# hiroharu-kato/neural_renderer

Measured on AMD Instinct MI355X. Metric: rasterize fwd+bwd Mpixels/sec @256x256 batch=64, higher is better.
Workload: dtype f32

## Files before the change

neural_renderer_amd/csrc/nr_device.h:

```cpp
#pragma once
#include <hip/hip_runtime.h>
#include <stdint.h>
#include <stdlib.h>

#include "../../include/nr_hip.h"

#define NR_API extern "C" __attribute__((visibility("default")))

namespace nr {

constexpr int WAVE = 64;


__device__ __forceinline__ bool is_backside(float x0, float y0, float x1, float y1, float x2, float y2)
{
    return (y2 - y0) * (x1 - x0) < (y1 - y0) * (x2 - x0);
}

__device__ __forceinline__ float to_pixel(float v, float fs) { return 0.5f * (v * fs + fs - 1.0f); }

__device__ __forceinline__ void compute_face_inv(const float px[3], const float py[3], float inv[9])
{
    inv[0] = py[1] - py[2];
    inv[1] = px[2] - px[1];
// ... 69 lines not shown
    if (thin || wild) {
        c.bw = S; c.n = S * S;
        return c;
    }
    const float xmin = fminf(fminf(px[0], px[1]), px[2]), xmax = fmaxf(fmaxf(px[0], px[1]), px[2]);
    const float ymin = fminf(fminf(py[0], py[1]), py[2]), ymax = fmaxf(fmaxf(py[0], py[1]), py[2]);
    const float lo_c = -2.0f, hi_c = (float)S + 1.0f;
    const int xl = max((int)ceilf(fminf(fmaxf(xmin - BBOX_GUARD, lo_c), hi_c)), 0);
    const int xh = min((int)floorf(fminf(fmaxf(xmax + BBOX_GUARD, lo_c), hi_c)), S - 1);
    const int yl = max((int)ceilf(fminf(fmaxf(ymin - BBOX_GUARD, lo_c), hi_c)), 0);
    const int yh = min((int)floorf(fminf(fmaxf(ymax + BBOX_GUARD, lo_c), hi_c)), S - 1);
    if (xl <= xh && yl <= yh) {
        c.x_lo = xl; c.y_lo = yl; c.bw = xh - xl + 1; c.n = c.bw * (yh - yl + 1);
    }
    return c;
}

__device__ __forceinline__ bool cand_pixel(const Cand &c, int i, int S, int &x, int &y)
{
    if (c.strip == 0) {
        const int yy = i / c.bw;
        x = c.x_lo + (i - yy * c.bw);
        y = c.y_lo + yy;
        return true;
    }
    const int m = i / STRIP_W, j = i - m * STRIP_W;
    const int o = (int)floorf(c.a * (float)m + c.b) - 1 + j;
    if (c.strip == 1) { y = m; x = o; } else { x = m; y = o; }
    return o >= 0 && o < S;
}

struct FaceLight {
    const float *light = nullptr;
    int tex_faces = 0;
    const float *textures = nullptr;
    float *grad_light = nullptr;
};

__device__ __forceinline__ int transpose_texel(int t, int ts)
{
    const int k = t % ts, j = (t / ts) % ts, i = t / (ts * ts);
    return (k * ts + j) * ts + i;
}

struct Taps {
    int isc[8];
    float w[8];
};

__device__ __forceinline__ void compute_taps(const float *__restrict__ z, const float *__restrict__ weight,
                                             float depth, int ts, double eps, Taps &t, bool flip = false)
{
    float tif[3];
    int ti[3];
    float fr[3];
#pragma unroll
    for (int k = 0; k < 3; k++) {
        float v = weight[k] * (float)(ts - 1) * (depth / z[k]);
        v = fmaxf(v, 0.0f);
        v = (float)fmin((double)v, (double)(ts - 1) - eps);
        tif[k] = v;
        ti[k] = (int)v;
        fr[k] = v - (float)ti[k];
    }
#pragma unroll
    for (int pn = 0; pn < 8; pn++) {
        float w = 1.0f;
        int idx[3];
#pragma unroll
        for (int k = 0; k < 3; k++) {
            if (((pn >> k) & 1) == 0) {
                w *= 1.0f - fr[k];
                idx[k] = ti[k];
            } else {
                w *= fr[k];
                idx[k] = ti[k] + 1;
            }
        }
        t.isc[pn] = (flip ? idx[2] : idx[0]) * ts * ts + idx[1] * ts + (flip ? idx[0] : idx[2]);
        t.w[pn] = w;
    }
}


__device__ __forceinline__ int f2i(float x) { return (int)x; }

__device__ __forceinline__ void texel_reads(const float *face, const float d[3], int H, int W, long long p[4], float w[4])
{
    const float pos_x = (face[0] * d[0] + face[2] * d[1] + face[4] * d[2]) * (float)(W - 1);
    const float pos_y = (face[1] * d[0] + face[3] * d[1] + face[5] * d[2]) * (float)(H - 1);
    const int xi = f2i(pos_x), yi = f2i(pos_y), yi1 = f2i(pos_y + 1.0f);
    const float wx1 = pos_x - (float)xi, wx0 = 1.0f - wx1;
    const float wy1 = pos_y - (float)yi, wy0 = 1.0f - wy1;
    const long long last = (long long)H * W - 1;
    auto clampi = [&](int row, int col) -> long long {
        const long long q = (long long)row * W + col;
        return q < 0 ? 0 : (q > last ? last : q);
    };
    p[0] = clampi(yi, xi);
    p[1] = clampi(yi1, xi);
    p[2] = clampi(yi, xi + 1);
    p[3] = clampi(yi1, xi + 1);
    w[0] = wx0 * wy0;
    w[1] = wx0 * wy1;
    w[2] = wx1 * wy0;
    w[3] = wx1 * wy1;
}

__device__ __forceinline__ int mirror_row(long long p, int H, int W)
{
    const int row = (int)(p / W), col = (int)(p - (long long)row * W);
    return (H - 1 - row) * W + col;
}

struct UVShade {
    const float *images = nullptr;
    const int32_t *table = nullptr;
    const float *faces_uv = nullptr;
    const int32_t *face_image = nullptr;
    const float *base = nullptr;
    int ts = 0, M = 0, P = 0;
    int shared = 0;
};

struct UVSample {
    int m, f0;
    int q[4];
    float w[4];
    Taps t;
};

__device__ __forceinline__ void corner_weights(const float (&z)[3], const float (&w)[3], float zp, float (&d)[3])
{
#pragma unroll
    for (int k = 0; k < 3; k++) d[k] = fminf(fmaxf(w[k] * (zp / z[k]), 0.0f), 1.0f);
}

__device__ __forceinline__ void uv_locate(const UVShade &uv, int fi, int tex_faces, const float *face, float w0, float w1,
                                          float w2, float zp, double eps, UVSample &s)
{
    const bool flip = fi >= tex_faces;
    s.f0 = flip ? fi - tex_faces : fi;
    const int m = uv.face_image[s.f0];
    s.m = (m >= 0 && m < uv.M) ? m : -1;
    const float fz[3] = {face[2], face[5], face[8]};
    const float w[3] = {w0, w1, w2};
    if (s.m < 0) {
        compute_taps(fz, w, zp, uv.ts, eps, s.t, flip);
        return;
    }
    float d[3];
#pragma unroll
    for (int k = 0; k < 3; k++) d[k] = fminf(fmaxf(w[k] * (zp / fz[k]), 0.0f), 1.0f);
    if (flip) {
        const float d0 = d[0];
        d[0] = d[2];
        d[2] = d0;
    }
    const int off = uv.table[3 * s.m], H = uv.table[3 * s.m + 1], W = uv.table[3 * s.m + 2];
    long long p[4];
    texel_reads(uv.faces_uv + (size_t)s.f0 * 6, d, H, W, p, s.w);
#pragma unroll
    for (int r = 0; r < 4; r++) s.q[r] = off + mirror_row(p[r], H, W);
}

__device__ __forceinline__ void uv_color(const UVShade &uv, const UVSample &s, int b, float c[3])
// ... 175 lines not shown
```

neural_renderer_amd/csrc/nr_forward.hip:

```cpp
#include "nr_device.h"

using namespace nr;

namespace {

constexpr size_t SMALL_LAUNCH_FACES = (size_t)16384 * 32;
constexpr int SMALL_AREA = 256;
constexpr int WAVE_AREA = 4096;
constexpr unsigned long long ZEMPTY = ~0ull;
constexpr int QSHARDS = 16;
constexpr int QSTRIDE = 32;

__device__ __forceinline__ unsigned depth_key(float zp)
{
    const unsigned u = __float_as_uint(zp + 0.0f);
    return (u & 0x80000000u) ? ~u : (u | 0x80000000u);
}

__device__ __forceinline__ unsigned long long zword(float zp, unsigned fn, int epoch)
{
    const unsigned long long k = depth_key(zp);
    return epoch < 0 ? (k << 32) | fn : ((unsigned long long)(unsigned)epoch << 56) | (k << 24) | fn;
}

struct FaceGeo {
    float x0, y0, z0, x1, y1, z1, x2, y2, z2, i0, i1, i2, i3, i4, i5, i6, i7, i8;
};

__device__ __forceinline__ bool inside_edges(const FaceGeo &q, float xp, float yp)
{
    return !(((yp - q.y0) * (q.x1 - q.x0) < (xp - q.x0) * (q.y1 - q.y0)) ||
             ((yp - q.y1) * (q.x2 - q.x1) < (xp - q.x1) * (q.y2 - q.y1)) ||
             ((yp - q.y2) * (q.x0 - q.x2) < (xp - q.x2) * (q.y0 - q.y2)));
}

__device__ __forceinline__ bool eval_inside(const FaceGeo &q, float xif, float yif, double near_d, double far_d, float &zp,
                                            float &w0, float &w1, float &w2)
{
    w0 = q.i0 * xif + q.i1 * yif + q.i2;
    w1 = q.i3 * xif + q.i4 * yif + q.i5;
    w2 = q.i6 * xif + q.i7 * yif + q.i8;
    w0 = fminf(fmaxf(w0, 0.0f), 1.0f);
    w1 = fminf(fmaxf(w1, 0.0f), 1.0f);
    w2 = fminf(fmaxf(w2, 0.0f), 1.0f);
    const float w_sum = (0.0f + w0) + w1 + w2;
    w0 /= w_sum;
    w1 /= w_sum;
    w2 /= w_sum;
    zp = 1.0f / (w0 / q.z0 + w1 / q.z1 + w2 / q.z2);
    if ((double)zp <= near_d || far_d <= (double)zp) return false;
    return zp < (float)far_d;
}

__device__ __forceinline__ bool eval_pixel(const FaceGeo &q, float xp, float yp, float xif, float yif, double near_d,
                                           double far_d, float &zp, float &w0, float &w1, float &w2)
{
    return inside_edges(q, xp, yp) && eval_inside(q, xif, yif, near_d, far_d, zp, w0, w1, w2);
}

__device__ __forceinline__ float pixel_center_f(int i, int S) { return (float)(2 * i + 1 - S) / (float)S; }
__device__ __forceinline__ float pixel_center_p(int i, int S, float inv_s, bool pow2)
{
    return pow2 ? (float)(2 * i + 1 - S) * inv_s : (float)(2 * i + 1 - S) / (float)S;
}

__device__ __forceinline__ void load_face_geo(const float *__restrict__ f, int S, FaceGeo &g, float inv[9])
{
    g.x0 = f[0]; g.y0 = f[1]; g.z0 = f[2]; g.x1 = f[3]; g.y1 = f[4]; g.z1 = f[5]; g.x2 = f[6]; g.y2 = f[7]; g.z2 = f[8];
    if (is_backside(g.x0, g.y0, g.x1, g.y1, g.x2, g.y2)) {
#pragma unroll
        for (int k = 0; k < 9; k++) inv[k] = 0.0f;
    } else {
        const float fs = (float)S;
        const float px[3] = {to_pixel(g.x0, fs), to_pixel(g.x1, fs), to_pixel(g.x2, fs)};
        const float py[3] = {to_pixel(g.y0, fs), to_pixel(g.y1, fs), to_pixel(g.y2, fs)};
        compute_face_inv(px, py, inv);
    }
    g.i0 = inv[0]; g.i1 = inv[1]; g.i2 = inv[2]; g.i3 = inv[3]; g.i4 = inv[4]; g.i5 = inv[5];
    g.i6 = inv[6]; g.i7 = inv[7]; g.i8 = inv[8];
}

constexpr int FR_ROWS = 128;
constexpr int FR_PIX = 256;
static_assert(SMALL_AREA <= 256, "rows and columns of a kept box are packed into 8 bits each");

template <int FACES>
struct FaceWaveLds {
    float g[18][FACES];
    int x_lo[FACES], y_lo[FACES], bw[FACES], img[FACES], fn[FACES];
    int rows[FR_ROWS];
    int pix[FR_PIX];
};

__device__ __forceinline__ int wave_inclusive_sum(int v)
{
    v += __builtin_amdgcn_update_dpp(0, v, 0x111, 0xf, 0xf, true);
    v += __builtin_amdgcn_update_dpp(0, v, 0x112, 0xf, 0xf, true);
    v += __builtin_amdgcn_update_dpp(0, v, 0x114, 0xf, 0xf, true);
    v += __builtin_amdgcn_update_dpp(0, v, 0x118, 0xf, 0xf, true);
    v += __builtin_amdgcn_update_dpp(0, v, 0x142, 0xa, 0xf, false);
    v += __builtin_amdgcn_update_dpp(0, v, 0x143, 0xc, 0xf, false);
    return v;
}

__device__ __forceinline__ void wave_lds_sync()
{
    __builtin_amdgcn_fence(__ATOMIC_RELEASE, "wavefront");
    __builtin_amdgcn_wave_barrier();
    __builtin_amdgcn_fence(__ATOMIC_ACQUIRE, "wavefront");
}

template <int FACES>
__device__ __forceinline__ bool slot_pixel(const FaceWaveLds<FACES> &L, int e, int S, double near_d, double far_d,
                                           unsigned long long *__restrict__ zbuf, unsigned long long &key,
                                           unsigned long long *&at, int epoch)
{
    const int s = e >> 16;
    FaceGeo q;
    q.z0 = L.g[6][s]; q.z1 = L.g[7][s]; q.z2 = L.g[8][s];
    q.i0 = L.g[9][s]; q.i1 = L.g[10][s]; q.i2 = L.g[11][s]; q.i3 = L.g[12][s]; q.i4 = L.g[13][s];
    q.i5 = L.g[14][s]; q.i6 = L.g[15][s]; q.i7 = L.g[16][s]; q.i8 = L.g[17][s];
    const int x = L.x_lo[s] + (e & 255), y = L.y_lo[s] + ((e >> 8) & 255);
    float zp, w0, w1, w2;
    const bool ok = eval_inside(q, (float)x, (float)y, near_d, far_d, zp, w0, w1, w2);
    key = zword(zp, (unsigned)L.fn[s], epoch);
    at = zbuf + ((size_t)L.img[s] * S + y) * S + x;
    return ok;
}


template <bool POW2, int FACES, int GROUP>
__global__ __launch_bounds__(256) void k_face_raster(const float *__restrict__ faces,
                                                     unsigned long long *__restrict__ zbuf,
                                                     int *__restrict__ large_list, int *__restrict__ wave_list,
                                                     int *__restrict__ n_large, int qcap, int nshards,
                                                     unsigned char *__restrict__ visible_faces, int n_faces_total, int F,
                                                     int S, double near_d, double far_d, int epoch,
                                                     unsigned char *__restrict__ touched)
{
    __shared__ FaceWaveLds<FACES> lds[4];
    FaceWaveLds<FACES> &L = lds[threadIdx.x >> 6];
    const int lane = threadIdx.x & 63;
    const int t = blockIdx.x * blockDim.x + threadIdx.x;
    if (t < n_faces_total && visible_faces) visible_faces[t] = 0;
    const int n_waves = (n_faces_total + FACES - 1) / FACES;
    const int i = ((lane / GROUP) * n_waves + (t >> 6)) * GROUP + (lane % GROUP);
    const bool live = lane < FACES && (t >> 6) < n_waves && i < n_faces_total;
    float f[9];
    {
        float *stage = &L.g[0][0];
        const size_t n_words = (size_t)n_faces_total * 9;
        constexpr int NLOAD = (9 * FACES + 63) / 64;
        float word[NLOAD];
#pragma unroll
        for (int k = 0; k < NLOAD; k++) {
            const int d = k * 64 + lane, run = d / (9 * GROUP), off = d - run * (9 * GROUP);
            const size_t src = ((size_t)run * n_waves + (t >> 6)) * (9 * GROUP) + off;
            const float v = faces[src < n_words ? src : n_words - 1];
            word[k] = src < n_words ? v : 0.0f;
        }
#pragma unroll
        for (int k = 0; k < NLOAD; k++) {
// ... 135 lines not shown
            const int e = queue[lane];
            const int rest = lane + 64 < waiting ? queue[lane + 64] : 0;
            wave_lds_sync();
            waiting -= 64;
            if (lane < waiting) queue[lane] = rest;
            evaluate(e);
        }
    }
    wave_lds_sync();
    if (lane < waiting) evaluate(queue[lane]);
    wave_lds_sync();
}

__device__ __forceinline__ int shard_first(int u, int s, int units, int nshards)
{
    const int start = (s * units) / nshards;
    return u >= start ? u - start : u - start + units;
}

__device__ __forceinline__ void wave_raster(const float *__restrict__ faces, unsigned long long *__restrict__ zbuf,
                                            const int *__restrict__ wave_list, const int cnt, int qcap, int nshards, int F, int S,
                                            double near_d, double far_d, int *__restrict__ queue, int epoch,
                                            unsigned char *__restrict__ touched)
{
    const int waves = gridDim.x * (blockDim.x >> 6), u = blockIdx.x * (blockDim.x >> 6) + (threadIdx.x >> 6);
    for (int s = 0; s < nshards; ++s) {
        const int n = __builtin_amdgcn_readlane(cnt, 2 * s + 1);
        for (int j = shard_first(u, s, waves, nshards); j < n; j += waves) {
            const int i = wave_list[(size_t)s * qcap + j];
            const float *f = faces + (size_t)i * 9;
            FaceGeo g;
            float inv[9];
            load_face_geo(f, S, g, inv);
            const Cand cd = face_candidates(g.x0, g.y0, g.x1, g.y1, g.x2, g.y2, S);
            const int b = i / F;
            raster_candidates(
                g, (unsigned)(i - b * F), cd.n, 0, 64,
                [&](int k, int &x, int &y) {
                    const int yy = k / cd.bw;
                    x = cd.x_lo + (k - yy * cd.bw);
                    y = cd.y_lo + yy;
                    return true;
                },
                queue, S, near_d, far_d, zbuf + (size_t)b * S * S, epoch, touched, (size_t)b * S * S);
        }
    }
}

__global__ __launch_bounds__(256) void k_large_raster(const float *__restrict__ faces,
                                                      unsigned long long *__restrict__ zbuf,
                                                      const int *__restrict__ large_list, const int *__restrict__ wave_list,
                                                      const int *__restrict__ n_large, int qcap, int nshards, int F, int S,
                                                      double near_d, double far_d, int epoch, unsigned char *__restrict__ touched)
{
    __shared__ int s_queue[4][CQ];
    __shared__ int s_cnt[2 * QSHARDS];
    int *queue = s_queue[threadIdx.x >> 6];
    int any = 0;
    if (threadIdx.x < 2 * QSHARDS) {
        any = s_cnt[threadIdx.x] = (int)threadIdx.x < 2 * nshards ? n_large[(threadIdx.x >> 1) * QSTRIDE + (threadIdx.x & 1)] + 1 : 0;
    }
    if (!__syncthreads_or(any)) return;
    const int cnt = s_cnt[threadIdx.x & (2 * QSHARDS - 1)];
    for (int s = 0; s < nshards; ++s) {
        const int n = __builtin_amdgcn_readlane(cnt, 2 * s);
        for (int j = shard_first((int)blockIdx.x, s, (int)gridDim.x, nshards); j < n; j += gridDim.x) {
            const int i = large_list[(size_t)s * qcap + j];
            const float *f = faces + (size_t)i * 9;
            FaceGeo g;
            float inv[9];
            load_face_geo(f, S, g, inv);
            const Cand cd = face_candidates(g.x0, g.y0, g.x1, g.y1, g.x2, g.y2, S);
            const int b = i / F;
            raster_candidates(
                g, (unsigned)(i - b * F), cd.n, (int)(threadIdx.x >> 6) * 64, 256,
                [&](int k, int &x, int &y) { return cand_pixel(cd, k, S, x, y); }, queue, S, near_d, far_d,
                zbuf + (size_t)b * S * S, epoch, touched, (size_t)b * S * S);
        }
    }
    wave_raster(faces, zbuf, wave_list, cnt, qcap, nshards, F, S, near_d, far_d, queue, epoch, touched);
}

enum ShadeMode { SHADE_CUBE = 0, SHADE_UV = 1, SHADE_CORNER = 2, SHADE_UV_SMOOTH = 3 };
template <int MODE>
__device__ __forceinline__ void shade_pixel(size_t i, int b, int fi, float w0, float w1, float w2, float depth,
                                            const float *__restrict__ faces, const float *__restrict__ zbase,
                                            const float *__restrict__ textures, float *__restrict__ rgb_map,
                                            int32_t *__restrict__ sampling_index_map,
                                            float *__restrict__ sampling_weight_map,
                                            const float *__restrict__ background, int bg_per_batch,
                                            float *__restrict__ alpha_map, int F, int ts, double eps, int fix_batch_z,
                                            const FaceLight &lit, const UVShade *uv = nullptr)
{
    if (alpha_map) alpha_map[i] = (fi >= 0) ? 1.0f : 0.0f;
    if (!rgb_map) return;
    float rgb[3];
    Taps t;
    constexpr bool UV = MODE == SHADE_UV || MODE == SHADE_UV_SMOOTH;
    if (MODE == SHADE_CORNER && fi >= 0) {
        const float *face = faces + ((size_t)b * F + fi) * 9;
        const float *cc = textures + ((size_t)b * F + fi) * 9;
        const float w[3] = {w0, w1, w2}, fz[3] = {face[2], face[5], face[8]};
        float d[3];
        corner_weights(fz, w, depth, d);
        const float *bg = background + (bg_per_batch ? 3 * b : 0);
#pragma unroll
        for (int c = 0; c < 3; c++) {
            rgb[c] = (cc[c] * d[0] + cc[3 + c] * d[1]) + cc[6 + c] * d[2];
            rgb[c] = rgb[c] * 1.0f + 0.0f * bg[c];
        }
    } else if (UV && fi >= 0) {
        UVSample s;
        uv_locate(*uv, fi, lit.tex_faces, faces + ((size_t)b * F + fi) * 9, w0, w1, w2, depth, eps, s);
        uv_color(*uv, s, b, rgb);
        if (MODE == SHADE_UV_SMOOTH) {
            const float *face = faces + ((size_t)b * F + fi) * 9;
            const float w[3] = {w0, w1, w2}, fz[3] = {face[2], face[5], face[8]};
            float e[3];
            corner_weights(fz, w, depth, e);
            const float *lc = lit.light + ((size_t)b * F + fi) * 9;
#pragma unroll
            for (int c = 0; c < 3; c++) rgb[c] *= (lc[c] * e[0] + lc[3 + c] * e[1]) + lc[6 + c] * e[2];
        } else {
            const float *lc = lit.light + ((size_t)b * F + fi) * 3;
            rgb[0] *= lc[0];
            rgb[1] *= lc[1];
            rgb[2] *= lc[2];
        }
        const float *bg = background + (bg_per_batch ? 3 * b : 0);
#pragma unroll
        for (int k = 0; k < 3; k++) rgb[k] = rgb[k] * 1.0f + 0.0f * bg[k];
    } else if (fi >= 0) {
        const float *face = (fix_batch_z ? faces + (size_t)b * F * 9 : zbase) + (size_t)fi * 9;
        const float *texture = textures + ((size_t)b * F + fi) * ts * ts * ts * 3;
        bool flip = false;
        if (lit.light) {
            flip = fi >= lit.tex_faces;
            texture = textures + ((size_t)b * lit.tex_faces + (flip ? fi - lit.tex_faces : fi)) * ts * ts * ts * 3;
        }
        const float w[3] = {w0, w1, w2};
        const float fz[3] = {face[2], face[5], face[8]};
        compute_taps(fz, w, depth, ts, eps, t, flip);
        rgb[0] = rgb[1] = rgb[2] = 0.0f;
#pragma unroll
        for (int pn = 0; pn < 8; pn++) {
            if (t.isc[pn] >= ts * ts * ts) continue;
            const float *tx = texture + t.isc[pn] * 3;
            rgb[0] += t.w[pn] * tx[0];
            rgb[1] += t.w[pn] * tx[1];
            rgb[2] += t.w[pn] * tx[2];
        }
        if (lit.light) {
            const float *lc = lit.light + ((size_t)b * F + fi) * 3;
            rgb[0] *= lc[0];
            rgb[1] *= lc[1];
            rgb[2] *= lc[2];
        }
        const float *bg = background + (bg_per_batch ? 3 * b : 0);
#pragma unroll
        for (int k = 0; k < 3; k++) rgb[k] = rgb[k] * 1.0f + 0.0f * bg[k];
    } else {
        const float *bg = background + (bg_per_batch ? 3 * b : 0);
#pragma unroll
        for (int k = 0; k < 3; k++) rgb[k] = 0.0f * 0.0f + 1.0f * bg[k];
#pragma unroll
        for (int pn = 0; pn < 8; pn++) { t.isc[pn] = 0; t.w[pn] = 0.0f; }
    }
    float *o = rgb_map + 3 * i;
    o[0] = rgb[0];
    o[1] = rgb[1];
    o[2] = rgb[2];
    if (MODE != SHADE_CUBE) return;
    if (sampling_index_map) {
        int4 *p = reinterpret_cast<int4 *>(sampling_index_map + 8 * i);
        p[0] = make_int4(t.isc[0], t.isc[1], t.isc[2], t.isc[3]);
        p[1] = make_int4(t.isc[4], t.isc[5], t.isc[6], t.isc[7]);
    }
    if (sampling_weight_map) {
        float4 *p = reinterpret_cast<float4 *>(sampling_weight_map + 8 * i);
        p[0] = make_float4(t.w[0], t.w[1], t.w[2], t.w[3]);
        p[1] = make_float4(t.w[4], t.w[5], t.w[6], t.w[7]);
    }
}

__global__ __launch_bounds__(256) void k_shade(const float *__restrict__ faces, const float *__restrict__ zbase,
                                               const float *__restrict__ textures,
                                               const int32_t *__restrict__ face_index_map,
                                               const float *__restrict__ weight_map,
                                               const float *__restrict__ depth_map, float *__restrict__ rgb_map,
                                               int32_t *__restrict__ sampling_index_map,
                                               float *__restrict__ sampling_weight_map,
                                               const float *__restrict__ background, int bg_per_batch,
                                               float *__restrict__ alpha_map, int F, int S, int ts, double eps,
                                               int fix_batch_z, size_t n_pixels, FaceLight lit)
{
    const size_t i = (size_t)blockIdx.x * blockDim.x + threadIdx.x;
    if (i >= n_pixels) return;
    const int fi = face_index_map[i];
    const int b = (int)(i / ((size_t)S * S));
    float w0 = 0.0f, w1 = 0.0f, w2 = 0.0f, depth = 0.0f;
    if (rgb_map && fi >= 0) { w0 = weight_map[3 * i]; w1 = weight_map[3 * i + 1]; w2 = weight_map[3 * i + 2]; depth = depth_map[i]; }
    shade_pixel<SHADE_CUBE>(i, b, fi, w0, w1, w2, depth, faces, zbase, textures, rgb_map, sampling_index_map, sampling_weight_map,
                            background, bg_per_batch, alpha_map, F, ts, eps, fix_batch_z, lit);
}

struct ResolveArgs {
    const float *faces;
    const unsigned long long *zbuf;
    int32_t *face_index_map;
    float *weight_map, *depth_map, *face_inv_map;
    unsigned char *visible_faces;
    int F, S;
    double near_d, far_d;
    size_t n_pixels;
    const float *zbase, *textures;
    float *rgb_map;
    const float *background;
    int bg_per_batch;
    float *alpha_map;
    int ts;
    double eps;
    int fix_batch_z, epoch;
    int *queue_counters;
    FaceLight lit;
    int sparse_weights;
    const unsigned char *touched;
};
struct ResolveArgsUV : ResolveArgs {
    UVShade uv;
};
template <int MODE> using ResolveArgsOf =
    typename std::conditional<MODE == SHADE_UV || MODE == SHADE_UV_SMOOTH, ResolveArgsUV, ResolveArgs>::type;

template <int MODE>
__device__ __forceinline__ void resolve_pixel(const ResolveArgsOf<MODE> &a, size_t i, bool drawn)
{
    const float *__restrict__ faces = a.faces;
    const int S = a.S, F = a.F, epoch = a.epoch;
    const unsigned long long pk = drawn ? a.zbuf[i] : ZEMPTY;
    int fn = -1;
    float zp = (float)a.far_d, w0 = 0.0f, w1 = 0.0f, w2 = 0.0f;
    float inv[9] = {0.0f, 0.0f, 0.0f, 0.0f, 0.0f, 0.0f, 0.0f, 0.0f, 0.0f};
    int b = 0;
    if (a.rgb_map || a.alpha_map) b = (int)(i / ((size_t)S * S));
    const bool hit = drawn && (epoch < 0 ? pk != ZEMPTY : (int)(pk >> 56) == epoch);
    if (hit) {
        fn = epoch < 0 ? (int)(unsigned)(pk & 0xffffffffu) : (int)(unsigned)(pk & 0xffffffu);
        const size_t SS = (size_t)S * S;
        b = (int)(i / SS);
        const int pn = (int)(i - (size_t)b * SS);
        const int py = pn / S, px = pn - py * S;
        FaceGeo g;
        load_face_geo(faces + ((size_t)b * F + fn) * 9, S, g, inv);
        eval_pixel(g, pixel_center_f(px, S), pixel_center_f(py, S), (float)px, (float)py, a.near_d, a.far_d, zp, w0, w1, w2);
        if (a.visible_faces) a.visible_faces[(size_t)b * F + fn] = 1;
    }
    a.face_index_map[i] = fn;
    if (a.depth_map) a.depth_map[i] = zp;
    if (a.weight_map && (hit || !a.sparse_weights)) {
        float *w = a.weight_map + 3 * i;
        w[0] = w0;
        w[1] = w1;
        w[2] = w2;
    }
    if (a.face_inv_map) {
        float *o = a.face_inv_map + 9 * i;
#pragma unroll
        for (int k = 0; k < 9; k++) o[k] = inv[k];
    }
    const UVShade *uv = nullptr;
    if constexpr (MODE == SHADE_UV || MODE == SHADE_UV_SMOOTH) uv = &a.uv;
    if (a.rgb_map || a.alpha_map)
        shade_pixel<MODE>(i, b, fn, w0, w1, w2, zp, faces, a.zbase, a.textures, a.rgb_map, nullptr, nullptr, a.background,
                          a.bg_per_batch, a.alpha_map, F, a.ts, a.eps, a.fix_batch_z, a.lit, uv);
}

__device__ __forceinline__ void reset_queue_counters(const ResolveArgs &a)
{
    if (blockIdx.x == 0 && threadIdx.x < QSHARDS && a.epoch >= 0) {
        a.queue_counters[threadIdx.x * QSTRIDE] = -1;
        a.queue_counters[threadIdx.x * QSTRIDE + 1] = -1;
    }
}

template <int MODE>
__global__ __launch_bounds__(256) void k_resolve(ResolveArgsOf<MODE> a)
{
    const size_t i = (size_t)blockIdx.x * blockDim.x + threadIdx.x;
    reset_queue_counters(a);
    if (i >= a.n_pixels) return;
    resolve_pixel<MODE>(a, i, !a.touched || a.touched[i >> 6] == (unsigned char)a.epoch);
}

template <int MODE>
__global__ __launch_bounds__(256) void k_resolve_quads(ResolveArgsOf<MODE> a)
{
    reset_queue_counters(a);
    const size_t i = (size_t)blockIdx.x * 256 + threadIdx.x, i0 = (size_t)blockIdx.x * 256 + 4 * threadIdx.x;
    const unsigned char ep = (unsigned char)a.epoch;
    unsigned char tq = ep, ti = (unsigned char)(ep + 1);
    if (threadIdx.x < 64 && i0 < a.n_pixels) tq = a.touched[i0 >> 6];
    if (i < a.n_pixels) ti = a.touched[i >> 6];
    if (tq != ep) {
        reinterpret_cast<int4 *>(a.face_index_map)[i0 >> 2] = make_int4(-1, -1, -1, -1);
        const float zf = (float)a.far_d;
        if (a.depth_map) reinterpret_cast<float4 *>(a.depth_map)[i0 >> 2] = make_float4(zf, zf, zf, zf);
        const float4 zero = make_float4(0.0f, 0.0f, 0.0f, 0.0f);
        if (a.weight_map && !a.sparse_weights) {
            float4 *w = reinterpret_cast<float4 *>(a.weight_map + 3 * i0);
            w[0] = zero; w[1] = zero; w[2] = zero;
        }
        if (a.face_inv_map) {
            float4 *o = reinterpret_cast<float4 *>(a.face_inv_map + 9 * i0);
#pragma unroll
            for (int k = 0; k < 9; k++) o[k] = zero;
        }
        if (a.alpha_map) reinterpret_cast<float4 *>(a.alpha_map)[i0 >> 2] = zero;
        if (a.rgb_map) {
            const float *bg = a.background + (a.bg_per_batch ? 3 * (int)(i0 / ((size_t)a.S * a.S)) : 0);
            float c[3];
#pragma unroll
            for (int k = 0; k < 3; k++) c[k] = 0.0f * 0.0f + 1.0f * bg[k];
            float4 *o = reinterpret_cast<float4 *>(a.rgb_map + 3 * i0);
            o[0] = make_float4(c[0], c[1], c[2], c[0]);
            o[1] = make_float4(c[1], c[2], c[0], c[1]);
            o[2] = make_float4(c[2], c[0], c[1], c[2]);
        }
    }
    if (ti == ep) resolve_pixel<MODE>(a, i, true);
}

}

NR_API int nr_version(void) { return NR_VERSION; }

NR_API const char *nr_error_string(int code)
{
    switch (code) {
        case 0: return "success";
        case NR_E_NULL: return "nr: a required pointer is NULL";
        case NR_E_SIZE: return "nr: size out of range";
        case NR_E_WORKSPACE: return "nr: workspace missing or too small";
        case NR_E_MODE: return "nr: nothing to do / inconsistent optional arguments";
        case NR_E_INDEX: return "nr: a vertex index lies outside [0, num_vertices)";
        default: return code > 0 ? hipGetErrorString((hipError_t)code) : "nr: unknown error";
    }
}

namespace {
struct FwdLayout {
    size_t zbuf_off, list_off, count_off, touch_off, total;
};
size_t queue_shard_capacity(size_t n_faces, int faces_per_wave, int nshards)
{
    const size_t per_wg = (size_t)4 * faces_per_wave, n_wg = (n_faces + per_wg - 1) / per_wg;
    return (n_wg + nshards - 1) / nshards * per_wg;
}

FwdLayout fwd_layout(int B, int F, int S)
{
    FwdLayout L;
    const size_t n = (size_t)B * F, P = (size_t)B * S * S;
    L.zbuf_off = 0;
    L.count_off = L.zbuf_off + P * sizeof(unsigned long long);
    L.list_off = align_up(L.count_off + (size_t)QSHARDS * QSTRIDE * sizeof(int), 256);
    L.touch_off = align_up(L.list_off + 2 * (n + (size_t)QSHARDS * 256) * sizeof(int), 256);
    L.total = L.touch_off + (P + 63) / 64;
    return L;
}
}

NR_API size_t nr_forward_workspace_bytes(int32_t B, int32_t F, int32_t S)
{
    if (check_sizes(B, F, S)) return 0;
    return fwd_layout(B, F, S).total;
}

namespace {
int run_forward(const float *faces, int32_t *face_index_map, float *weight_map, float *depth_map, float *face_inv_map,
                unsigned char *visible_faces, int B, int F, int S, double near, double far, void *workspace,
                size_t workspace_bytes, hipStream_t st, const float *faces_z_ref, const float *textures, float *rgb_map,
                const float *background, int bg_per_batch, float *alpha_map, int ts, double eps, int fix_batch_z,
                int flags = 0, const FaceLight &lit = FaceLight(), const UVShade *uv = nullptr, bool corner = false,
                bool corner_light = false)
{
    if (!faces || !face_index_map) return NR_E_NULL;
    if (int e = check_sizes(B, F, S)) return e;
    const FwdLayout L = fwd_layout(B, F, S);
    if (!workspace || workspace_bytes < L.total) return NR_E_WORKSPACE;
    const size_t n = (size_t)B * F, P = (size_t)B * S * S;
    unsigned char *ws = (unsigned char *)workspace;
    unsigned long long *zbuf = (unsigned long long *)(ws + L.zbuf_off);
    int *n_large = (int *)(ws + L.count_off);
    int *large_list = (int *)(ws + L.list_off);

    int epoch = -1;
    if ((flags & NR_FLAG_ZBUF_EPOCH) && F < (1 << 24)) {
        epoch = (flags >> 8) & 0xff;
        if (epoch > 254) return NR_E_MODE;
    } else {
        if (int he = fill_bytes(zbuf, 0xff, P * sizeof(unsigned long long) + (size_t)QSHARDS * QSTRIDE * sizeof(int), st)) return he;
    }
    const bool small_launch = n < SMALL_LAUNCH_FACES;
    const int nshards = small_launch ? 1 : QSHARDS;
    const int qcap = (int)queue_shard_capacity(n, small_launch ? 16 : 64, nshards);
    int *wave_list = large_list + (size_t)nshards * qcap;
    unsigned char *touched = epoch >= 0 ? ws + L.touch_off : nullptr;
    {
        const bool pow2 = (S & (S - 1)) == 0, small = small_launch;
#define NR_FACE_RASTER(P, FC, G)                                                                                           \
    hipLaunchKernelGGL((k_face_raster<P, FC, G>), dim3((unsigned)((n + 4 * FC - 1) / (4 * FC))), dim3(256), 0, st, faces, zbuf, \
                       large_list, wave_list, n_large, qcap, nshards, visible_faces, (int)n, F, S, near, far, epoch, touched)
        if (small) { if (pow2) NR_FACE_RASTER(true, 16, 4); else NR_FACE_RASTER(false, 16, 4); }
        else { if (pow2) NR_FACE_RASTER(true, 64, 16); else NR_FACE_RASTER(false, 64, 16); }
#undef NR_FACE_RASTER
    }
    const unsigned queue_wgs = (unsigned)(n / 256 < 256 ? 256 : (n / 256 > 2048 ? 2048 : n / 256));
    hipLaunchKernelGGL(k_large_raster, dim3(queue_wgs), dim3(256), 0, st, faces, zbuf, large_list, wave_list, n_large, qcap, nshards,
                       F, S, near, far, epoch, touched);
    ResolveArgs ra;
    ra.faces = faces; ra.zbuf = zbuf; ra.face_index_map = face_index_map; ra.weight_map = weight_map; ra.depth_map = depth_map;
    ra.face_inv_map = face_inv_map; ra.visible_faces = visible_faces; ra.F = F; ra.S = S; ra.near_d = near; ra.far_d = far;
    ra.n_pixels = P; ra.zbase = faces_z_ref ? faces_z_ref : faces; ra.textures = textures; ra.rgb_map = rgb_map;
    ra.background = background; ra.bg_per_batch = bg_per_batch; ra.alpha_map = alpha_map; ra.ts = ts; ra.eps = eps;
    ra.fix_batch_z = fix_batch_z; ra.epoch = epoch; ra.queue_counters = n_large; ra.lit = lit;
    ra.sparse_weights = (flags & NR_FLAG_SPARSE_WEIGHT_MAP) ? 1 : 0; ra.touched = touched;
    const uintptr_t align = (uintptr_t)face_index_map | (uintptr_t)weight_map | (uintptr_t)depth_map | (uintptr_t)face_inv_map |
                            (uintptr_t)rgb_map | (uintptr_t)alpha_map;
    const bool quads = touched && S % 2 == 0 && (align & 15) == 0;
    const dim3 grid((unsigned)((P + 255) / 256));
    if (uv) {
        ResolveArgsUV rau;
        static_cast<ResolveArgs &>(rau) = ra;
        rau.uv = *uv;
        if (corner_light) {
            if (quads) hipLaunchKernelGGL(k_resolve_quads<SHADE_UV_SMOOTH>, grid, dim3(256), 0, st, rau);
            else hipLaunchKernelGGL(k_resolve<SHADE_UV_SMOOTH>, grid, dim3(256), 0, st, rau);
        } else if (quads) {
            hipLaunchKernelGGL(k_resolve_quads<SHADE_UV>, grid, dim3(256), 0, st, rau);
        } else {
            hipLaunchKernelGGL(k_resolve<SHADE_UV>, grid, dim3(256), 0, st, rau);
        }
    } else if (corner) {
        if (quads) hipLaunchKernelGGL(k_resolve_quads<SHADE_CORNER>, grid, dim3(256), 0, st, ra);
        else hipLaunchKernelGGL(k_resolve<SHADE_CORNER>, grid, dim3(256), 0, st, ra);
    } else if (quads) {
        hipLaunchKernelGGL(k_resolve_quads<SHADE_CUBE>, grid, dim3(256), 0, st, ra);
    } else {
        hipLaunchKernelGGL(k_resolve<SHADE_CUBE>, grid, dim3(256), 0, st, ra);
    }
    return launch_status();
}
}

NR_API int nr_forward_face_index_map(const float *faces, int32_t *face_index_map, float *weight_map, float *depth_map,
                                     float *face_inv_map, uint8_t *visible_faces, int32_t B, int32_t F, int32_t S,
                                     double near, double far, void *workspace, size_t workspace_bytes, void *stream)
{
    return run_forward(faces, face_index_map, weight_map, depth_map, face_inv_map, visible_faces, B, F, S, near, far,
                       workspace, workspace_bytes, (hipStream_t)stream, nullptr, nullptr, nullptr, nullptr, 0, nullptr, 0,
                       0.0, 0);
}

NR_API int nr_forward_rasterize(const float *faces, const float *faces_z_ref, const float *textures,
                                int32_t *face_index_map, float *weight_map, float *depth_map, float *rgb_map,
                                float *alpha_map, uint8_t *visible_faces, const float *background, int32_t bg_per_batch,
                                int32_t B, int32_t F, int32_t S, int32_t ts, double near, double far, double eps,
                                int32_t flags, void *workspace, size_t workspace_bytes, void *stream)
{
    return nr_forward_rasterize_lit(nullptr, faces, faces_z_ref, textures, face_index_map, weight_map, depth_map, rgb_map,
                                    alpha_map, visible_faces, background, bg_per_batch, B, F, S, ts, near, far, eps, flags,
                                    workspace, workspace_bytes, stream);
}

int nr::face_light_args(const nr_face_light *lit, int F, bool backward, FaceLight &out)
{
    out = FaceLight();
    if (!lit) return 0;
    if (!lit->light) return NR_E_NULL;
    if (lit->texture_faces < 1 || (lit->texture_faces != F && 2 * (int64_t)lit->texture_faces != F)) return NR_E_SIZE;
    out.light = lit->light;
    out.tex_faces = lit->texture_faces;
    if (backward) {
        out.textures = lit->textures;
        out.grad_light = lit->grad_light;
        if (out.grad_light && !out.textures) return NR_E_NULL;
    }
    return 0;
}

NR_API int nr_forward_rasterize_lit(const nr_face_light *lit, const float *faces, const float *faces_z_ref,
                                    const float *textures, int32_t *face_index_map, float *weight_map, float *depth_map,
                                    float *rgb_map, float *alpha_map, uint8_t *visible_faces, const float *background,
                                    int32_t bg_per_batch, int32_t B, int32_t F, int32_t S, int32_t ts, double near,
                                    double far, double eps, int32_t flags, void *workspace, size_t workspace_bytes,
                                    void *stream)
{
    if (rgb_map) {
        if (!textures || !background) return NR_E_NULL;
        if (ts < 2 || ts > 1024) return NR_E_SIZE;
    }
    FaceLight fl;
    if (int e = face_light_args(rgb_map ? lit : nullptr, F, false, fl)) return e;
    return run_forward(faces, face_index_map, weight_map, depth_map, nullptr, visible_faces, B, F, S, near, far,
                       workspace, workspace_bytes, (hipStream_t)stream, faces_z_ref, textures, rgb_map, background,
                       bg_per_batch, alpha_map, ts, eps, (flags & NR_FLAG_FIX_TEXTURE_BATCH_Z) ? 1 : 0, flags, fl);
}

int nr::uv_images_args(const nr_face_light *lit, const nr_uv_images *uv, int B, int F, FaceLight &fl, UVShade &out)
{
    out = UVShade();
    if (!lit || !uv) return NR_E_NULL;
    if (int e = face_light_args(lit, F, false, fl)) return e;
    fl.grad_light = lit->grad_light;
    if (!uv->images || !uv->image_table || !uv->faces_uv || !uv->face_image || !uv->base) return NR_E_NULL;
    if (uv->texture_size < 2 || uv->texture_size > 1024 || uv->num_images < 1 || uv->num_pixels < 1 ||
        uv->num_pixels > 0x7ffffffe)
        return NR_E_SIZE;
    if (uv->image_batch != 1 && uv->image_batch != B) return NR_E_SIZE;
    out.images = uv->images;
    out.table = uv->image_table;
    out.faces_uv = uv->faces_uv;
    out.face_image = uv->face_image;
    out.base = uv->base;
    out.ts = uv->texture_size;
    out.M = uv->num_images;
    out.P = uv->num_pixels;
    out.shared = uv->image_batch == 1 ? 1 : 0;
// ... 74 lines not shown
```

Baseline: 15060.

## Restructure resolve shading: hoist loads, specialize ts=2 cube texture path

Resolve kernels now issue the zbuf, touched and background loads early, and load face vertices into registers before computing geometry. Cube-mode shading is inlined into resolve_pixel with an early-issued texture fetch. A ts=2 specialization loads the whole 24-float texture as six float4s, and texture tap loads are made branchless. Launch bounds add an occupancy hint of 8. The aim is to hide memory latency in the resolve pass, at the cost of more registers and extra code paths.

Result: faster. 15370 (median of 6 runs) (+2.0%).

```diff
diff --git a/neural_renderer_amd/csrc/nr_device.h b/neural_renderer_amd/csrc/nr_device.h
--- a/neural_renderer_amd/csrc/nr_device.h
+++ b/neural_renderer_amd/csrc/nr_device.h
@@ -175,6 +175,30 @@
     }
 }
 
+__device__ __forceinline__ void sum_taps(const float *__restrict__ texture, const Taps &t, int T, float c[3])
+{
+    float tx[8][3];
+    unsigned inside = 0;
+#pragma unroll
+    for (int pn = 0; pn < 8; pn++) {
+        inside |= (unsigned)(t.isc[pn] < T) << pn;
+        const float *p = texture + min(t.isc[pn], T - 1) * 3;
+        tx[pn][0] = p[0];
+        tx[pn][1] = p[1];
+        tx[pn][2] = p[2];
+    }
+    c[0] = c[1] = c[2] = 0.0f;
+#pragma unroll
+    for (int pn = 0; pn < 8; pn++) {
+        const bool in = (inside >> pn) & 1u;
+#pragma unroll
+        for (int k = 0; k < 3; k++) {
+            const float s = c[k] + t.w[pn] * tx[pn][k];
+            c[k] = in ? s : c[k];
+        }
+    }
+}
+
 
 __device__ __forceinline__ int f2i(float x) { return (int)x; }
 
diff --git a/neural_renderer_amd/csrc/nr_forward.hip b/neural_renderer_amd/csrc/nr_forward.hip
--- a/neural_renderer_amd/csrc/nr_forward.hip
+++ b/neural_renderer_amd/csrc/nr_forward.hip
@@ -64,7 +64,7 @@
     return pow2 ? (float)(2 * i + 1 - S) * inv_s : (float)(2 * i + 1 - S) / (float)S;
 }
 
-__device__ __forceinline__ void load_face_geo(const float *__restrict__ f, int S, FaceGeo &g, float inv[9])
+__device__ __forceinline__ void face_geo(const float (&f)[9], int S, FaceGeo &g, float inv[9])
 {
     g.x0 = f[0]; g.y0 = f[1]; g.z0 = f[2]; g.x1 = f[3]; g.y1 = f[4]; g.z1 = f[5]; g.x2 = f[6]; g.y2 = f[7]; g.z2 = f[8];
     if (is_backside(g.x0, g.y0, g.x1, g.y1, g.x2, g.y2)) {
@@ -78,6 +78,11 @@
     }
     g.i0 = inv[0]; g.i1 = inv[1]; g.i2 = inv[2]; g.i3 = inv[3]; g.i4 = inv[4]; g.i5 = inv[5];
     g.i6 = inv[6]; g.i7 = inv[7]; g.i8 = inv[8];
+}
+__device__ __forceinline__ void load_face_geo(const float *__restrict__ f, int S, FaceGeo &g, float inv[9])
+{
+    const float v[9] = {f[0], f[1], f[2], f[3], f[4], f[5], f[6], f[7], f[8]};
+    face_geo(v, S, g, inv);
 }
 
 constexpr int FR_ROWS = 128;
@@ -379,13 +384,96 @@
 }
 
 enum ShadeMode { SHADE_CUBE = 0, SHADE_UV = 1, SHADE_CORNER = 2, SHADE_UV_SMOOTH = 3 };
+__device__ __forceinline__ void load_background(const float *__restrict__ background, int bg_per_batch, int b, float (&bg)[3])
+{
+    const float *p = background + (bg_per_batch ? 3 * b : 0);
+    bg[0] = p[0];
+    bg[1] = p[1];
+    bg[2] = p[2];
+}
+
+template <bool TS2>
+struct CubeFace {
+    float fz[3], lc[3];
+    const float *texture;
+    bool flip;
+    float4 cube[TS2 ? 6 : 1];
+};
+
+template <bool TS2>
+__device__ __forceinline__ void load_cube_face(CubeFace<TS2> &c, int b, int fi, const float *__restrict__ faces,
+                                               const float *__restrict__ zbase, const float *__restrict__ textures, int F,
+                                               int ts, int fix_batch_z, const FaceLight &lit)
+{
+    const float *face = (fix_batch_z ? faces + (size_t)b * F * 9 : zbase) + (size_t)fi * 9;
+    c.fz[0] = face[2]; c.fz[1] = face[5]; c.fz[2] = face[8];
+    if constexpr (TS2) {
+        c.flip = false;
+        c.texture = textures + ((size_t)b * F + fi) * 24;
+    } else {
+        c.flip = lit.light && fi >= lit.tex_faces;
+        c.texture = textures + ((size_t)b * (lit.light ? lit.tex_faces : F) + (c.flip ? fi - lit.tex_faces : fi)) * ts * ts * ts * 3;
+        const float *lc = lit.light ? lit.light + ((size_t)b * F + fi) * 3 : face;
+        c.lc[0] = lc[0]; c.lc[1] = lc[1]; c.lc[2] = lc[2];
+    }
+}
+
+__device__ __forceinline__ void load_cube(CubeFace<true> &c)
+{
+#pragma unroll
+    for (int k = 0; k < 6; k++) c.cube[k] = reinterpret_cast<const float4 *>(c.texture)[k];
+}
+__device__ __forceinline__ void load_cube(CubeFace<false> &) {}
+
+__device__ __forceinline__ float quad_elem(const float4 &q, int k) { return k == 0 ? q.x : (k == 1 ? q.y : (k == 2 ? q.z : q.w)); }
+
+__device__ __forceinline__ void store_taps(const Taps &t, int32_t *__restrict__ sampling_index_map,
+                                           float *__restrict__ sampling_weight_map, size_t i)
+{
+    if (sampling_index_map) {
+        int4 *p = reinterpret_cast<int4 *>(sampling_index_map + 8 * i);
+        p[0] = make_int4(t.isc[0], t.isc[1], t.isc[2], t.isc[3]);
+        p[1] = make_int4(t.isc[4], t.isc[5], t.isc[6], t.isc[7]);
+    }
+    if (sampling_weight_map) {
+        float4 *p = reinterpret_cast<float4 *>(sampling_weight_map + 8 * i);
+        p[0] = make_float4(t.w[0], t.w[1], t.w[2], t.w[3]);
+        p[1] = make_float4(t.w[4], t.w[5], t.w[6], t.w[7]);
+    }
+}
+
+template <bool TS2>
+__device__ __forceinline__ void shade_cube(const CubeFace<TS2> &c, const float (&w)[3], float depth, int ts, double eps,
+                                           bool lit, Taps &t, float (&rgb)[3], int32_t *__restrict__ sampling_index_map = nullptr,
+                                           float *__restrict__ sampling_weight_map = nullptr, size_t i = 0)
+{
+    compute_taps(c.fz, w, depth, ts, eps, t, c.flip);
+    store_taps(t, sampling_index_map, sampling_weight_map, i);
+    if constexpr (TS2) {
+        rgb[0] = rgb[1] = rgb[2] = 0.0f;
+#pragma unroll
+        for (int pn = 0; pn < 8; pn++) {
+            const int b0 = pn & 1, b1 = (pn >> 1) & 1, b2 = pn >> 2;
+            const int e = (b0 * 4 + b1 * 2 + b2) * 3;
+#pragma unroll
+            for (int k = 0; k < 3; k++) rgb[k] += t.w[pn] * quad_elem(c.cube[(e + k) >> 2], (e + k) & 3);
+        }
+    } else {
+        sum_taps(c.texture, t, ts * ts * ts, rgb);
+    }
+    if (!TS2 && lit) {
+        rgb[0] *= c.lc[0];
+        rgb[1] *= c.lc[1];
+        rgb[2] *= c.lc[2];
+    }
+}
+
 template <int MODE>
 __device__ __forceinline__ void shade_pixel(size_t i, int b, int fi, float w0, float w1, float w2, float depth,
                                             const float *__restrict__ faces, const float *__restrict__ zbase,
                                             const float *__restrict__ textures, float *__restrict__ rgb_map,
                                             int32_t *__restrict__ sampling_index_map,
-                                            float *__restrict__ sampling_weight_map,
-                                            const float *__restrict__ background, int bg_per_batch,
+                                            float *__restrict__ sampling_weight_map, const float (&bg)[3],
                                             float *__restrict__ alpha_map, int F, int ts, double eps, int fix_batch_z,
                                             const FaceLight &lit, const UVShade *uv = nullptr)
 {
@@ -400,7 +488,6 @@
         const float w[3] = {w0, w1, w2}, fz[3] = {face[2], face[5], face[8]};
         float d[3];
         corner_weights(fz, w, depth, d);
-        const float *bg = background + (bg_per_batch ? 3 * b : 0);
 #pragma unroll
         for (int c = 0; c < 3; c++) {
             rgb[c] = (cc[c] * d[0] + cc[3 + c] * d[1]) + cc[6 + c] * d[2];
@@ -424,40 +511,16 @@
             rgb[1] *= lc[1];
             rgb[2] *= lc[2];
         }
-        const float *bg = background + (bg_per_batch ? 3 * b : 0);
 #pragma unroll
         for (int k = 0; k < 3; k++) rgb[k] = rgb[k] * 1.0f + 0.0f * bg[k];
     } else if (fi >= 0) {
-        const float *face = (fix_batch_z ? faces + (size_t)b * F * 9 : zbase) + (size_t)fi * 9;
-        const float *texture = textures + ((size_t)b * F + fi) * ts * ts * ts * 3;
-        bool flip = false;
-        if (lit.light) {
-            flip = fi >= lit.tex_faces;
-            texture = textures + ((size_t)b * lit.tex_faces + (flip ? fi - lit.tex_faces : fi)) * ts * ts * ts * 3;
-        }
+        CubeFace<false> c;
+        load_cube_face(c, b, fi, faces, zbase, textures, F, ts, fix_batch_z, lit);
         const float w[3] = {w0, w1, w2};
-        const float fz[3] = {face[2], face[5], face[8]};
-        compute_taps(fz, w, depth, ts, eps, t, flip);
-        rgb[0] = rgb[1] = rgb[2] = 0.0f;
-#pragma unroll
-        for (int pn = 0; pn < 8; pn++) {
-            if (t.isc[pn] >= ts * ts * ts) continue;
-            const float *tx = texture + t.isc[pn] * 3;
-            rgb[0] += t.w[pn] * tx[0];
-            rgb[1] += t.w[pn] * tx[1];
-            rgb[2] += t.w[pn] * tx[2];
-        }
-        if (lit.light) {
-            const float *lc = lit.light + ((size_t)b * F + fi) * 3;
-            rgb[0] *= lc[0];
-            rgb[1] *= lc[1];
-            rgb[2] *= lc[2];
-        }
-        const float *bg = background + (bg_per_batch ? 3 * b : 0);
+        shade_cube(c, w, depth, ts, eps, lit.light != nullptr, t, rgb, sampling_index_map, sampling_weight_map, i);
 #pragma unroll
         for (int k = 0; k < 3; k++) rgb[k] = rgb[k] * 1.0f + 0.0f * bg[k];
     } else {
-        const float *bg = background + (bg_per_batch ? 3 * b : 0);
 #pragma unroll
         for (int k = 0; k < 3; k++) rgb[k] = 0.0f * 0.0f + 1.0f * bg[k];
 #pragma unroll
@@ -467,17 +530,7 @@
     o[0] = rgb[0];
     o[1] = rgb[1];
     o[2] = rgb[2];
-    if (MODE != SHADE_CUBE) return;
-    if (sampling_index_map) {
-        int4 *p = reinterpret_cast<int4 *>(sampling_index_map + 8 * i);
-        p[0] = make_int4(t.isc[0], t.isc[1], t.isc[2], t.isc[3]);
-        p[1] = make_int4(t.isc[4], t.isc[5], t.isc[6], t.isc[7]);
-    }
-    if (sampling_weight_map) {
-        float4 *p = reinterpret_cast<float4 *>(sampling_weight_map + 8 * i);
-        p[0] = make_float4(t.w[0], t.w[1], t.w[2], t.w[3]);
-        p[1] = make_float4(t.w[4], t.w[5], t.w[6], t.w[7]);
-    }
+    if (MODE == SHADE_CUBE && fi < 0) store_taps(t, sampling_index_map, sampling_weight_map, i);
 }
 
 __global__ __launch_bounds__(256) void k_shade(const float *__restrict__ faces, const float *__restrict__ zbase,
@@ -493,12 +546,14 @@
 {
     const size_t i = (size_t)blockIdx.x * blockDim.x + threadIdx.x;
     if (i >= n_pixels) return;
+    const int b = (int)(i / ((size_t)S * S));
+    float bg[3] = {0.0f, 0.0f, 0.0f};
+    if (rgb_map) load_background(background, bg_per_batch, b, bg);
     const int fi = face_index_map[i];
-    const int b = (int)(i / ((size_t)S * S));
     float w0 = 0.0f, w1 = 0.0f, w2 = 0.0f, depth = 0.0f;
     if (rgb_map && fi >= 0) { w0 = weight_map[3 * i]; w1 = weight_map[3 * i + 1]; w2 = weight_map[3 * i + 2]; depth = depth_map[i]; }
     shade_pixel<SHADE_CUBE>(i, b, fi, w0, w1, w2, depth, faces, zbase, textures, rgb_map, sampling_index_map, sampling_weight_map,
-                            background, bg_per_batch, alpha_map, F, ts, eps, fix_batch_z, lit);
+                            bg, alpha_map, F, ts, eps, fix_batch_z, lit);
 }
 
 struct ResolveArgs {
@@ -529,28 +584,47 @@
 template <int MODE> using ResolveArgsOf =
     typename std::conditional<MODE == SHADE_UV || MODE == SHADE_UV_SMOOTH, ResolveArgsUV, ResolveArgs>::type;
 
-template <int MODE>
-__device__ __forceinline__ void resolve_pixel(const ResolveArgsOf<MODE> &a, size_t i, bool drawn)
-{
+template <int MODE, bool TS2>
+__device__ __forceinline__ void resolve_pixel(const ResolveArgsOf<MODE> &a, size_t i, unsigned long long pk, const float (&bg)[3])
+{
+    constexpr bool CUBE = MODE == SHADE_CUBE;
     const float *__restrict__ faces = a.faces;
     const int S = a.S, F = a.F, epoch = a.epoch;
-    const unsigned long long pk = drawn ? a.zbuf[i] : ZEMPTY;
     int fn = -1;
     float zp = (float)a.far_d, w0 = 0.0f, w1 = 0.0f, w2 = 0.0f;
-    float inv[9] = {0.0f, 0.0f, 0.0f, 0.0f, 0.0f, 0.0f, 0.0f, 0.0f, 0.0f};
     int b = 0;
-    if (a.rgb_map || a.alpha_map) b = (int)(i / ((size_t)S * S));
-    const bool hit = drawn && (epoch < 0 ? pk != ZEMPTY : (int)(pk >> 56) == epoch);
+    float rgb[3];
+    const bool hit = epoch < 0 ? pk != ZEMPTY : (int)(pk >> 56) == epoch;
     if (hit) {
         fn = epoch < 0 ? (int)(unsigned)(pk & 0xffffffffu) : (int)(unsigned)(pk & 0xffffffu);
         const size_t SS = (size_t)S * S;
         b = (int)(i / SS);
         const int pn = (int)(i - (size_t)b * SS);
         const int py = pn / S, px = pn - py * S;
+        const float *f = faces + ((size_t)b * F + fn) * 9;
+        const float fv[9] = {f[0], f[1], f[2], f[3], f[4], f[5], f[6], f[7], f[8]};
+        CubeFace<TS2> c;
+        if (CUBE && a.rgb_map) load_cube_face(c, b, fn, faces, a.zbase, a.textures, F, a.ts, a.fix_batch_z, a.lit);
         FaceGeo g;
-        load_face_geo(faces + ((size_t)b * F + fn) * 9, S, g, inv);
+        float inv[9];
+        face_geo(fv, S, g, inv);
+        if (CUBE && a.rgb_map) load_cube(c);
         eval_pixel(g, pixel_center_f(px, S), pixel_center_f(py, S), (float)px, (float)py, a.near_d, a.far_d, zp, w0, w1, w2);
-        if (a.visible_faces) a.visible_faces[(size_t)b * F + fn] = 1;
+        if (a.face_inv_map) {
+            float *o = a.face_inv_map + 9 * i;
+#pragma unroll
+            for (int k = 0; k < 9; k++) o[k] = inv[k];
+        }
+        if (CUBE && a.rgb_map) {
+            Taps t;
+            const float w[3] = {w0, w1, w2};
+            shade_cube(c, w, zp, a.ts, a.eps, a.lit.light != nullptr, t, rgb);
+#pragma unroll
+            for (int k = 0; k < 3; k++) rgb[k] = rgb[k] * 1.0f + 0.0f * bg[k];
+        }
+    } else {
+#pragma unroll
+        for (int k = 0; k < 3; k++) rgb[k] = 0.0f * 0.0f + 1.0f * bg[k];
     }
     a.face_index_map[i] = fn;
     if (a.depth_map) a.depth_map[i] = zp;
@@ -560,16 +634,26 @@
         w[1] = w1;
         w[2] = w2;
     }
-    if (a.face_inv_map) {
+    if (a.face_inv_map && !hit) {
         float *o = a.face_inv_map + 9 * i;
 #pragma unroll
-        for (int k = 0; k < 9; k++) o[k] = inv[k];
-    }
-    const UVShade *uv = nullptr;
-    if constexpr (MODE == SHADE_UV || MODE == SHADE_UV_SMOOTH) uv = &a.uv;
-    if (a.rgb_map || a.alpha_map)
-        shade_pixel<MODE>(i, b, fn, w0, w1, w2, zp, faces, a.zbase, a.textures, a.rgb_map, nullptr, nullptr, a.background,
-                          a.bg_per_batch, a.alpha_map, F, a.ts, a.eps, a.fix_batch_z, a.lit, uv);
+        for (int k = 0; k < 9; k++) o[k] = 0.0f;
+    }
+    if (hit && a.visible_faces) a.visible_faces[(size_t)b * F + fn] = 1;
+    if constexpr (CUBE) {
+        if (a.alpha_map) a.alpha_map[i] = hit ? 1.0f : 0.0f;
+        if (a.rgb_map) {
+            float *o = a.rgb_map + 3 * i;
+            o[0] = rgb[0];
+            o[1] = rgb[1];
+            o[2] = rgb[2];
+        }
+    } else if (a.rgb_map || a.alpha_map) {
+        const UVShade *uv = nullptr;
+        if constexpr (MODE == SHADE_UV || MODE == SHADE_UV_SMOOTH) uv = &a.uv;
+        shade_pixel<MODE>(i, b, fn, w0, w1, w2, zp, faces, a.zbase, a.textures, a.rgb_map, nullptr, nullptr, bg, a.alpha_map, F,
+                          a.ts, a.eps, a.fix_batch_z, a.lit, uv);
+    }
 }
 
 __device__ __forceinline__ void reset_queue_counters(const ResolveArgs &a)
@@ -581,23 +665,32 @@
 }
 
 template <int MODE>
-__global__ __launch_bounds__(256) void k_resolve(ResolveArgsOf<MODE> a)
+__global__ __launch_bounds__(256, 8) void k_resolve(ResolveArgsOf<MODE> a)
 {
     const size_t i = (size_t)blockIdx.x * blockDim.x + threadIdx.x;
     reset_queue_counters(a);
     if (i >= a.n_pixels) return;
-    resolve_pixel<MODE>(a, i, !a.touched || a.touched[i >> 6] == (unsigned char)a.epoch);
-}
-
-template <int MODE>
-__global__ __launch_bounds__(256) void k_resolve_quads(ResolveArgsOf<MODE> a)
+    float bg[3] = {0.0f, 0.0f, 0.0f};
+    if (a.rgb_map) load_background(a.background, a.bg_per_batch, a.bg_per_batch ? (int)(i / ((size_t)a.S * a.S)) : 0, bg);
+    const bool drawn = !a.touched || a.touched[i >> 6] == (unsigned char)a.epoch;
+    resolve_pixel<MODE, false>(a, i, drawn ? a.zbuf[i] : ZEMPTY, bg);
+}
+
+template <int MODE, bool TS2 = false>
+__global__ __launch_bounds__(256, 8) void k_resolve_quads(ResolveArgsOf<MODE> a)
 {
     reset_queue_counters(a);
     const size_t i = (size_t)blockIdx.x * 256 + threadIdx.x, i0 = (size_t)blockIdx.x * 256 + 4 * threadIdx.x;
+    const size_t last = a.n_pixels - 1;
     const unsigned char ep = (unsigned char)a.epoch;
-    unsigned char tq = ep, ti = (unsigned char)(ep + 1);
-    if (threadIdx.x < 64 && i0 < a.n_pixels) tq = a.touched[i0 >> 6];
-    if (i < a.n_pixels) ti = a.touched[i >> 6];
+    const bool filler = threadIdx.x < 64 && i0 < a.n_pixels;
+    const unsigned char tq_read = a.touched[(filler ? i0 : min(i, last)) >> 6], ti_read = a.touched[min(i, last) >> 6];
+    float bg[3] = {0.0f, 0.0f, 0.0f};
+    if (a.rgb_map)
+        load_background(a.background, a.bg_per_batch, a.bg_per_batch ? (int)(((size_t)blockIdx.x * 256) / ((size_t)a.S * a.S)) : 0, bg);
+    const unsigned char tq = filler ? tq_read : ep, ti = i < a.n_pixels ? ti_read : (unsigned char)(ep + 1);
+    unsigned long long pk = ZEMPTY;
+    if (ti == ep) pk = a.zbuf[i];
     if (tq != ep) {
         reinterpret_cast<int4 *>(a.face_index_map)[i0 >> 2] = make_int4(-1, -1, -1, -1);
         const float zf = (float)a.far_d;
@@ -614,7 +707,6 @@
         }
         if (a.alpha_map) reinterpret_cast<float4 *>(a.alpha_map)[i0 >> 2] = zero;
         if (a.rgb_map) {
-            const float *bg = a.background + (a.bg_per_batch ? 3 * (int)(i0 / ((size_t)a.S * a.S)) : 0);
             float c[3];
 #pragma unroll
             for (int k = 0; k < 3; k++) c[k] = 0.0f * 0.0f + 1.0f * bg[k];
@@ -624,7 +716,7 @@
             o[2] = make_float4(c[2], c[0], c[1], c[2]);
         }
     }
-    if (ti == ep) resolve_pixel<MODE>(a, i, true);
+    if (ti == ep) resolve_pixel<MODE, TS2>(a, i, pk, bg);
 }
 
 }
@@ -724,7 +816,7 @@
     ra.sparse_weights = (flags & NR_FLAG_SPARSE_WEIGHT_MAP) ? 1 : 0; ra.touched = touched;
     const uintptr_t align = (uintptr_t)face_index_map | (uintptr_t)weight_map | (uintptr_t)depth_map | (uintptr_t)face_inv_map |
                             (uintptr_t)rgb_map | (uintptr_t)alpha_map;
-    const bool quads = touched && S % 2 == 0 && (align & 15) == 0;
+    const bool quads = touched && S % 2 == 0 && (align & 15) == 0 && (!(rgb_map && bg_per_batch) || ((size_t)S * S) % 256 == 0);
     const dim3 grid((unsigned)((P + 255) / 256));
     if (uv) {
         ResolveArgsUV rau;
@@ -741,6 +833,8 @@
     } else if (corner) {
         if (quads) hipLaunchKernelGGL(k_resolve_quads<SHADE_CORNER>, grid, dim3(256), 0, st, ra);
         else hipLaunchKernelGGL(k_resolve<SHADE_CORNER>, grid, dim3(256), 0, st, ra);
+    } else if (quads && rgb_map && !lit.light && ts == 2 && (float)(1.0 - eps) < 1.0f && ((uintptr_t)textures & 15) == 0) {
+        hipLaunchKernelGGL((k_resolve_quads<SHADE_CUBE, true>), grid, dim3(256), 0, st, ra);
     } else if (quads) {
         hipLaunchKernelGGL(k_resolve_quads<SHADE_CUBE>, grid, dim3(256), 0, st, ra);
     } else {
```
